# alexbuburuzan/MObI

Measured on AMD Instinct MI355X. Metric: denoising throughput (UNet element-forwards/s = steps/s x UNet batch), higher is better.
Workload: dtype bf16; 1 GPU; mobi_nusc_512 UNet denoising step, 8 objects/GPU (UNet batch 16), latent 64x64, DDIM-50 schedule, cfg_scale 1.0; objects_per_gpu=8, unet_batch=16, latent=64, sampler=ddim, parallelism=dp1 (objects sharded, no collective in the loop)

## Files before the change

mobi_amd/csrc/igemm.hip:

```cpp
#include <stdlib.h>

#include <type_traits>

#include "common.h"
#include "tuning.h"
#include "igemm_small.h"

#ifndef MOBI_FRAG2
#define MOBI_FRAG2 0
#endif
#ifndef MOBI_DMA_KS
#define MOBI_DMA_KS 1
#endif
#if defined(MOBI_IGEMM_FENCE) && MOBI_IGEMM_FENCE
#define MOBI_SCHED_FENCE() __builtin_amdgcn_sched_barrier(0)
#else
#define MOBI_SCHED_FENCE() ((void)0)
#endif

#ifndef MOBI_DBG_SKIP
#define MOBI_DBG_SKIP 0
#endif
#ifndef MOBI_PP_DMA_KS
#define MOBI_PP_DMA_KS 1
// ... 515 lines not shown

template <typename T, int NT, bool GEGLU, bool VEC = true>
__device__ __forceinline__ int direct_epilogue(const IgemmArgs& a, f32x4 (&acc)[NT][4], DirectEpiRegs<NT>& q, int lane,
                                               int group, int nw0, int mw0) {
  const int r16 = lane & 15, g4 = lane >> 4;
  const float scale = a.scale;
  T* __restrict__ outT = reinterpret_cast<T*>(a.out);
  const bool has_vec = VEC && (a.bias || a.rowvec);
  if (has_vec) {
#pragma unroll
    for (int ni = 0; ni < NT; ++ni) asm volatile("" : "+v"(q.bias[ni]));
  }
  if (!GEGLU && a.residual) {
#pragma unroll
    for (int ni = 0; ni < NT; ++ni) { asm volatile("" : "+v"(q.res[ni][0])); asm volatile("" : "+v"(q.res[ni][1])); }
  }
  constexpr bool geglu = GEGLU;
#pragma unroll
  for (int p = 0; p < 2; ++p) {
    const int mi = geglu ? 2 * p + (g4 >> 1) : 2 * p + (g4 & 1);
    const int m = mw0 + mi * 16 + r16;
    const int img = m / a.hw_out, rem = m - img * a.hw_out;
    T* rowp = outT + (long long)(group * a.imgs_per_group + img) * a.out_img_stride + (long long)rem * a.cout;
#pragma unroll
    for (int ni = 0; ni < NT; ++ni) {
      f32x4 x = acc[ni][2 * p] * scale, y = acc[ni][2 * p + 1] * scale;
      if (has_vec) {
        const f32x4 b = __builtin_bit_cast(f32x4, q.bias[ni]);
        x += b; y += b;
      }
      float xs[4] = {x[0], x[1], x[2], x[3]}, ys[4] = {y[0], y[1], y[2], y[3]};
      if constexpr (geglu) MOBI_SWAP4("v_permlane32_swap_b32", xs, ys);
      else MOBI_SWAP4("v_permlane16_swap_b32", xs, ys);
      if constexpr (geglu) {
        float o[4];
#pragma unroll
        for (int r = 0; r < 4; ++r) o[r] = xs[r] * gelu_erf_f(ys[r]);
        vm_store8(rowp + (nw0 >> 1) + ni * 8 + 4 * (g4 & 1), pack4<T>(o));
      } else {
        float o[8] = {xs[0], xs[1], xs[2], xs[3], ys[0], ys[1], ys[2], ys[3]};
        if (a.residual) {
          float rf[8];
          unpack8<T>(q.res[ni][p], rf);
#pragma unroll
          for (int j = 0; j < 8; ++j) o[j] += rf[j];
        }
        vm_store16(rowp + nw0 + ni * 16 + 8 * (g4 >> 1), pack8<T>(o));
      }
    }
  }
  return 2 * NT;
}

template <typename T, int NT, bool GEGLU>
__device__ __forceinline__ void ring_register_epilogue(const IgemmArgs& a, f32x4 (&acc)[NT][8], int lane, int group, int nw0,
                                                       int mw0) {
  const int r16 = lane & 15, g4 = lane >> 4;
  T* __restrict__ outT = reinterpret_cast<T*>(a.out);
  const T* __restrict__ resid = reinterpret_cast<const T*>(a.residual);
  const bool has_res = !GEGLU && a.residual;
  u32x4 res[2][NT];
#pragma unroll
  for (int ni = 0; ni < NT; ++ni) res[0][ni] = res[1][ni] = u32x4{0u, 0u, 0u, 0u};
  auto out_row = [&](int k) {
    const int mi = GEGLU ? 2 * k + (g4 >> 1) : 2 * k + (g4 & 1);
    return mw0 + mi * 16 + r16;
  };
  auto request_res = [&](int k, u32x4 (&r)[NT]) {
    const int m = out_row(k);
    const int img = m / a.hw_out, rem = m - img * a.hw_out;
    const T* rowp = resid + (long long)(group * a.imgs_per_group + img) * a.res_img_stride + (long long)rem * a.cout + nw0 +
                    8 * (g4 >> 1);
#pragma unroll
    for (int ni = 0; ni < NT; ++ni) r[ni] = vm_load16(rowp + ni * 16);
  };
  if (has_res) request_res(0, res[0]);
#pragma unroll
  for (int k = 0; k < 4; ++k) {
    if (has_res) {
      if (k + 1 < 4) request_res(k + 1, res[(k + 1) & 1]);
      const bool both = k > 0 && k + 1 < 4;
      if (both) { if (NT == 5) asm volatile("s_waitcnt vmcnt(10)" ::: "memory"); else asm volatile("s_waitcnt vmcnt(8)" ::: "memory"); }
      else                  { if (NT == 5) asm volatile("s_waitcnt vmcnt(5)" ::: "memory"); else asm volatile("s_waitcnt vmcnt(4)" ::: "memory"); }
    }
    if constexpr (!GEGLU) {
#pragma unroll
      for (int ni = 0; ni < NT; ++ni) asm volatile("" : "+v"(res[k & 1][ni]));
    }
    const int m = out_row(k);
    const int img = m / a.hw_out, rem = m - img * a.hw_out;
    T* rowp = outT + (long long)(group * a.imgs_per_group + img) * a.out_img_stride + (long long)rem * a.cout;
#pragma unroll
    for (int ni = 0; ni < NT; ++ni) {
      const f32x4 x = acc[ni][2 * k], y = acc[ni][2 * k + 1];
      float xs[4] = {x[0], x[1], x[2], x[3]}, ys[4] = {y[0], y[1], y[2], y[3]};
      if constexpr (GEGLU) MOBI_SWAP4("v_permlane32_swap_b32", xs, ys);
      else MOBI_SWAP4("v_permlane16_swap_b32", xs, ys);
      if constexpr (GEGLU) {
        float o[4];
#pragma unroll
        for (int r = 0; r < 4; ++r) o[r] = xs[r] * gelu_erf_f(ys[r]);
        vm_store8(rowp + (nw0 >> 1) + ni * 8 + 4 * (g4 & 1), pack4<T>(o));
      } else {
        float o[8] = {xs[0], xs[1], xs[2], xs[3], ys[0], ys[1], ys[2], ys[3]};
        if (has_res) {
          float rf[8];
          unpack8<T>(res[k & 1][ni], rf);
#pragma unroll
          for (int j = 0; j < 8; ++j) o[j] += rf[j];
        }
        vm_store16(rowp + nw0 + ni * 16 + 8 * (g4 >> 1), pack8<T>(o));
      }
    }
  }
}

template <int NT>
struct PpEpiRegs {
  u32x4 res0[NT];
};
template <typename T, int NT>
__device__ __forceinline__ void pp_residual_request(const IgemmArgs& a, u32x4 (&r)[NT], int p, int lane, int group,
                                                    int nw0, int mw0) {
  const int r16 = lane & 15, g4 = lane >> 4;
  const T* __restrict__ resid = reinterpret_cast<const T*>(a.residual);
  const int m = mw0 + (2 * p + (g4 & 1)) * 16 + r16;
  const int img = m >> a.hw_shift, rem = m & (a.hw_out - 1);
  const T* rowp = resid + (long long)(group * a.imgs_per_group + img) * a.res_img_stride + (long long)rem * a.cout +
                  nw0 + 8 * (g4 >> 1);
#pragma unroll
  for (int ni = 0; ni < NT; ++ni) r[ni] = vm_load16(rowp + ni * 16);
}
#ifndef MOBI_PP_RES0_EARLY
#define MOBI_PP_RES0_EARLY 0
#endif
template <typename T, int NT, bool GEGLU>
__device__ __forceinline__ int pp_epilogue_request(const IgemmArgs& a, PpEpiRegs<NT>& q, int lane, int group, int nw0,
                                                   int mw0) {
  if (!MOBI_PP_RES0_EARLY || GEGLU || !a.residual) return 0;
  pp_residual_request<T, NT>(a, q.res0, 0, lane, group, nw0, mw0);
  return NT;
}
template <typename T, int NT, bool GEGLU>
__device__ __forceinline__ int pp_epilogue(const IgemmArgs& a, f32x4 (&acc)[NT][4], PpEpiRegs<NT>& q, int lane, int group,
                                           int nw0, int mw0) {
  const int r16 = lane & 15, g4 = lane >> 4;
  T* __restrict__ outT = reinterpret_cast<T*>(a.out);
  const bool resid = !GEGLU && a.residual;
  u32x4 res1[NT];
  int n_issued = 0;
  if (resid) {
    if (!MOBI_PP_RES0_EARLY) {
      pp_residual_request<T, NT>(a, q.res0, 0, lane, group, nw0, mw0);
      n_issued += NT;
    }
    pp_residual_request<T, NT>(a, res1, 1, lane, group, nw0, mw0);
    n_issued += NT;
    if (!MOBI_PP_RES0_EARLY) {
      if (NT == 5) asm volatile("s_waitcnt vmcnt(5)" ::: "memory"); else asm volatile("s_waitcnt vmcnt(4)" ::: "memory");
    }
#pragma unroll
    for (int ni = 0; ni < NT; ++ni) asm volatile("" : "+v"(q.res0[ni]));
  }
#pragma unroll
// ... 954 lines not shown
  MOBI_STAMP_AT(2);
  wait_vmcnt_le(vm_issued - mk_req);
  finish_tile(p_nw0, p_mw0);
  if constexpr (SLAB) {
    if (a.sync) {
      const int L = xcd_remap(blockIdx.x, nblk);
      MOBI_TILE_OF_M(L, ftm, ftn);
      splitk_arrive_and_finish<T, 512>(a, L, ftm * BM, BM, ftn * BN, BN, &s_arrive);
    }
  }
#if MOBI_STAMP
  asm volatile("s_waitcnt vmcnt(0)" ::: "memory");
  MOBI_STAMP_AT(3);
  if (g_stamps && threadIdx.x == 0) {
    unsigned long long* d = g_stamps + (size_t)(blockIdx.x + gridDim.x * (blockIdx.y + gridDim.y * blockIdx.z)) * 8;
    d[5] = (unsigned long long)nk;
    d[6] = (unsigned long long)((nblk - (int)blockIdx.x + (int)gridDim.x - 1) / (int)gridDim.x);
  }
#endif
#if MOBI_STAMP == 3
  if (g_phase && lane == 0) {
    unsigned long long* d = g_phase + ((size_t)(blockIdx.x + gridDim.x * (blockIdx.y + gridDim.y * blockIdx.z)) * 8 + wave) * 16;
    for (int i = 0; i < 8; ++i) d[i] = pp_acc[i >> 2][i & 3];
    d[8] = pp_n;
  }
#endif
#undef MOBI_PP_T
#undef MOBI_PP_BARRIER
}

typedef _Float16 f16x2_t __attribute__((ext_vector_type(2)));
typedef __bf16 bf16x2_t __attribute__((ext_vector_type(2)));
__device__ __forceinline__ void rowstat_acc(const f16x8& x, float& sum, float& sq) {
  struct Q { f16x2_t p[4]; };
  const Q q = __builtin_bit_cast(Q, x);
  const f16x2_t one = {(_Float16)1.0f, (_Float16)1.0f};
#pragma unroll
  for (int i = 0; i < 4; ++i) {
    sum = __builtin_amdgcn_fdot2(q.p[i], one, sum, false);
    sq = __builtin_amdgcn_fdot2(q.p[i], q.p[i], sq, false);
  }
}
__device__ __forceinline__ void rowstat_acc(const bf16x8& x, float& sum, float& sq) {
  struct Q { bf16x2_t p[4]; };
  const Q q = __builtin_bit_cast(Q, x);
  const bf16x2_t one = {(__bf16)1.0f, (__bf16)1.0f};
#pragma unroll
  for (int i = 0; i < 4; ++i) {
    sum = __builtin_amdgcn_fdot2_f32_bf16(q.p[i], one, sum, false);
    sq = __builtin_amdgcn_fdot2_f32_bf16(q.p[i], q.p[i], sq, false);
  }
}

template <int NT, int MT, int SPW>
__device__ __forceinline__ void ln_fold_acc(const IgemmArgs& a, f32x4 (&acc)[NT][MT], const float (&ls_sum)[SPW],
                                            const float (&ls_sq)[SPW], float* s_rowstat, int lane, int wm, int wn, int nw0,
                                            bool add_bias) {
  const int r16 = lane & 15, g4 = lane >> 4;
  const float inv_k = 1.0f / (float)a.ktot;
#pragma unroll
  for (int i = 0; i < SPW; ++i) {
    float sm = ls_sum[i], sq = ls_sq[i];
    sm += __shfl_xor(sm, 16, 64); sq += __shfl_xor(sq, 16, 64);
    sm += __shfl_xor(sm, 32, 64); sq += __shfl_xor(sq, 32, 64);
    const float mean = sm * inv_k;
    const float var = fmaxf(sq * inv_k - mean * mean, 0.f);
    if (g4 == 0) {
      float* d = s_rowstat + ((wm * MT + SPW * wn + i) * 16 + r16) * 2;
      d[0] = mean; d[1] = rsqrtf(var + a.ln_eps);
    }
  }
  __syncthreads();
#pragma unroll
  for (int ni = 0; ni < NT; ++ni) {
    const int n = nw0 + ni * 16 + g4 * 4;
    f32x4 sv = f32x4{0.f, 0.f, 0.f, 0.f}, bv = f32x4{0.f, 0.f, 0.f, 0.f};
    if (n < a.n_packed) {
      sv = *reinterpret_cast<const f32x4*>(a.ln_svec + n);
      if (add_bias && a.bias) bv = *reinterpret_cast<const f32x4*>(a.bias + n);
    }
#pragma unroll
    for (int mi = 0; mi < MT; ++mi) {
      const float* d = s_rowstat + ((wm * MT + mi) * 16 + r16) * 2;
      const float mean = d[0], rstd = d[1];
      acc[ni][mi] = rstd * (acc[ni][mi] - mean * sv) + bv;
    }
  }
}

template <typename T, int NT, bool TR, int NW, int MT, bool LNF = false, bool LEAKY = false>
__global__ __launch_bounds__(NW * 64, 2) void igemm_ring_kernel(const IgemmArgs a) {
  typedef typename Vec8<T>::type frag_t;
  constexpr bool WIDE = NW == 8;
  constexpr int BM = 2 * MT * 16;
  constexpr int APW = BM / 16 / NW;
  constexpr int WAVE_N = NT * 16;
  constexpr int BN = (NW / 2) * WAVE_N;
  constexpr int WPIECES = BN / 16;
  constexpr int SLOT = (BM + BN) * 64;
  constexpr int RING = 4 * SLOT;
  constexpr int STAGE_BYTES = EpiGeom<32, TR, NT>::BYTES;
  constexpr int LDS_BYTES = RING > NW * STAGE_BYTES ? RING : NW * STAGE_BYTES;
  constexpr unsigned OOB = 0x80000000u;
  __shared__ __attribute__((aligned(16))) unsigned char lds[LDS_BYTES];
  __shared__ int s_arrive;
  __shared__ float s_rowstat[LNF ? BM * 2 : 2];
  static_assert(!(LNF && TR), "the LayerNorm fold has no transposed-output form");
  typedef __attribute__((address_space(3))) void* lds_ptr_t;

  const int tid = threadIdx.x, lane = tid & 63, wave = tid >> 6;
  const int wave_s = __builtin_amdgcn_readfirstlane(wave);
  const int wm = wave & 1, wn = wave >> 1;
  const int group = blockIdx.z;
  const int nblk = a.tiles_m * a.tiles_n;
  const int L = xcd_remap(blockIdx.x, nblk);
  MOBI_TILE_OF(L, tile_m, tile_n);
  const int m0 = tile_m * BM, n0 = tile_n * BN;
  constexpr int SPW = MT / (NW / 2);
  constexpr bool lnf = LNF;
  float ls_sum[SPW], ls_sq[SPW];
#pragma unroll
  for (int i = 0; i < SPW; ++i) ls_sum[i] = ls_sq[i] = 0.f;
  MOBI_STAMP_AT(0);
  const bool w_tiled = a.w_tiled != nullptr;
  const T* wgt = (w_tiled ? reinterpret_cast<const T*>(a.w_tiled) : reinterpret_cast<const T*>(a.weight)) + (long long)group * a.w_group_stride;
  const __amdgpu_buffer_rsrc_t rx0 = __builtin_amdgcn_make_buffer_rsrc(const_cast<void*>(a.src0), 0, a.src0_bytes, 0x00020000);
  const __amdgpu_buffer_rsrc_t rx1 =
      __builtin_amdgcn_make_buffer_rsrc(const_cast<void*>(a.src1 ? a.src1 : a.src0), 0, a.src1 ? a.src1_bytes : 0, 0x00020000);
  const __amdgpu_buffer_rsrc_t rw = __builtin_amdgcn_make_buffer_rsrc(const_cast<T*>(wgt), 0, a.w_bytes, 0x00020000);

  const int rp = lane >> 2;
  const unsigned perm = (0x1320u >> (((rp >> 2) & 3) * 4)) & 3u;
  const unsigned chunk16 = (((unsigned)lane & 3u) ^ perm) * 16u;
  int x_base[APW], x_h[APW], x_w[APW];
  bool x_ok[APW];
#pragma unroll
  for (int j = 0; j < APW; ++j) {
    const int m = m0 + 16 * (APW * wave + j) + rp;
    x_ok[j] = m < a.M;
    const int mm = x_ok[j] ? m : 0;
    const int img = mm / a.hw_out, rem = mm - img * a.hw_out;
    const int ho = rem / a.wout, wo = rem - ho * a.wout;
    x_base[j] = (group * a.imgs_per_group + img) * a.img_pix_stride;
    x_h[j] = ho * a.stride - a.pad_h;
    x_w[j] = wo * a.stride - a.pad_w;
  }
  unsigned w_off[3];
#pragma unroll
  for (int i = 0; i < 3; ++i) {
    const int piece = wave + NW * i;
    const int n = n0 + 16 * piece + rp;
    w_off[i] = (piece < WPIECES && n < a.n_packed) ? (unsigned)n * (unsigned)a.ktot * 2u + chunk16 : OOB;
    if (w_tiled) w_off[i] = (piece < WPIECES && n0 + 16 * piece < a.n_packed)
                                ? (unsigned)(n0 / 16 + piece) * (unsigned)(a.ktot >> 5) * 1024u + (unsigned)lane * 16u : OOB;
  }
  const int hlog = a.hin << a.up, wlog = a.win << a.up;
  const int ks_all = a.ktot >> 5;
  const int ks_begin = blockIdx.y * a.nk_per * 2;
  const int ks_end = min(ks_all, ks_begin + a.nk_per * 2);
  int u_c, u_tap, u_ky, u_kx;
  {
    const long long c_first = (long long)ks_begin * 32;
    u_tap = (int)(c_first / a.C); u_c = (int)(c_first - (long long)u_tap * a.C);
    u_ky = u_tap / a.kw; u_kx = u_tap - u_ky * a.kw;
  }
  unsigned f_row[APW];
#pragma unroll
  for (int j = 0; j < APW; ++j) f_row[j] = OOB;
  int f_tap = -1, f_src = -1, f_ks = ks_begin;

  auto issue_step = [&]() {
    unsigned char* st = lds + (f_ks & 3) * SLOT;
    const bool live = f_ks < ks_end;
    const int src = u_c >= a.c0 ? 1 : 0;
    if (live && (u_tap != f_tap || src != f_src)) {
      f_tap = u_tap; f_src = src;
      const unsigned cs2 = (unsigned)(src ? a.c1 : a.c0) * 2u;
#pragma unroll
      for (int j = 0; j < APW; ++j) {
        const int hi = x_h[j] + u_ky, wi = x_w[j] + u_kx;
        const bool ok = x_ok[j] && (unsigned)hi < (unsigned)hlog && (unsigned)wi < (unsigned)wlog;
        f_row[j] = ok ? (unsigned)(x_base[j] + (hi >> a.up) * a.win + (wi >> a.up)) * cs2 + chunk16 : OOB;
      }
    }
    const int soff = (src ? u_c - a.c0 : u_c) * 2;
#pragma unroll
    for (int j = 0; j < APW; ++j) {
      const unsigned vo = live ? f_row[j] : OOB;
      if (src) __builtin_amdgcn_raw_ptr_buffer_load_lds(rx1, (lds_ptr_t)(st + 16 * (APW * wave_s + j) * 64), 16, vo, soff, 0, 0);
      else     __builtin_amdgcn_raw_ptr_buffer_load_lds(rx0, (lds_ptr_t)(st + 16 * (APW * wave_s + j) * 64), 16, vo, soff, 0, 0);
    }
    const int kb = w_tiled ? f_ks * 1024 : f_ks * 64;
#pragma unroll
    for (int i = 0; i < 3; ++i) {
      if (i == 2 && (NT != 5 || wave_s >= NW / 2)) break;
      const unsigned vo = live ? w_off[i] : OOB;
      __builtin_amdgcn_raw_ptr_buffer_load_lds(rw, (lds_ptr_t)(st + BM * 64 + (wave_s + NW * i) * 1024), 16, vo, kb, 0, 0);
    }
    ++f_ks;
    if (live) {
      u_c += 32;
      if (u_c >= a.C) { u_c = 0; ++u_tap; if (++u_kx == a.kw) { u_kx = 0; ++u_ky; } }
    }
  };
  auto wait_step = [&]() {
    if (NT == 5 && wave_s < NW / 2) {
      if (APW == 2) asm volatile("s_waitcnt vmcnt(10)" ::: "memory"); else asm volatile("s_waitcnt vmcnt(8)" ::: "memory");
    } else {
      if (APW == 2) asm volatile("s_waitcnt vmcnt(8)" ::: "memory"); else asm volatile("s_waitcnt vmcnt(6)" ::: "memory");
    }
  };

  f32x4 acc[NT][MT];
#pragma unroll
  for (int i = 0; i < NT; ++i)
#pragma unroll
    for (int j = 0; j < MT; ++j) acc[i][j] = f32x4{0.f, 0.f, 0.f, 0.f};

  const int r16 = lane & 15, g4 = lane >> 4;
  if constexpr (WIDE && MT == 8 && !TR) {
    if (!lnf && a.ring_direct && (a.bias || a.rowvec)) {
      const float* vec = a.bias;
      if (a.rowvec) {
        const int img = __builtin_amdgcn_readfirstlane((m0 + wm * 128) / a.hw_out);
        vec = a.rowvec + (long long)(group * a.imgs_per_group + img) * a.rowvec_stride;
      }
#pragma unroll
      for (int i = 0; i < NT; ++i) {
        const f32x4 b = *reinterpret_cast<const f32x4*>(vec + n0 + wn * WAVE_N + i * 16 + g4 * 4);
#pragma unroll
        for (int j = 0; j < MT; ++j) acc[i][j] = b;
      }
    }
  }
  const unsigned fsw = (((unsigned)g4 ^ ((0x1320u >> (((r16 >> 2) & 3) * 4)) & 3u)) << 4);
  const unsigned char* xrd = lds + (wm * MT * 16 + r16) * 64 + fsw;
  const unsigned char* wrd = lds + BM * 64 + (wn * WAVE_N + r16) * 64 + fsw;

  auto read_frags = [&](int s, frag_t (&xf)[MT], frag_t (&wf)[NT]) {
    const int so = (s & 3) * SLOT;
#pragma unroll
    for (int mi = 0; mi < MT; ++mi) xf[mi] = __builtin_bit_cast(frag_t, ld16(xrd + so + mi * 16 * 64));
#pragma unroll
    for (int ni = 0; ni < NT; ++ni) wf[ni] = __builtin_bit_cast(frag_t, ld16(wrd + so + ni * 16 * 64));
  };
  auto multiply = [&](const frag_t (&xf)[MT], const frag_t (&wf)[NT]) {
    __builtin_amdgcn_s_setprio(1);
#pragma unroll
    for (int ni = 0; ni < NT; ++ni)
#pragma unroll
      for (int mi = 0; mi < MT; ++mi)
        acc[ni][mi] = TR ? mfma16(xf[mi], wf[ni], acc[ni][mi]) : mfma16(wf[ni], xf[mi], acc[ni][mi]);
    __builtin_amdgcn_s_setprio(0);
  };
  auto multiply_stats = [&](const frag_t (&xf)[MT], const frag_t (&wf)[NT], auto wnc) {
    constexpr int WNC = decltype(wnc)::value;
    __builtin_amdgcn_s_setprio(1);
#pragma unroll
    for (int ni = 0; ni < NT; ++ni)
#pragma unroll
      for (int mi = 0; mi < MT; ++mi) {
        acc[ni][mi] = TR ? mfma16(xf[mi], wf[ni], acc[ni][mi]) : mfma16(wf[ni], xf[mi], acc[ni][mi]);
        if (ni == 0 && mi < SPW) rowstat_acc(xf[SPW * WNC + mi], ls_sum[mi], ls_sq[mi]);
      }
#pragma unroll
    for (int i = 0; i < 8 * SPW; ++i) {
      __builtin_amdgcn_sched_group_barrier(0x008, 2, 0);
      __builtin_amdgcn_sched_group_barrier(0x002, 1, 0);
    }
#pragma unroll
    for (int i = 0; i < SPW; ++i) asm volatile("" : "+v"(ls_sum[i]), "+v"(ls_sq[i]));
    __builtin_amdgcn_s_setprio(0);
  };
#define MOBI_RING_BARRIER()                   \
  do {                                        \
    __builtin_amdgcn_sched_barrier(0);        \
    __builtin_amdgcn_s_barrier();             \
    __builtin_amdgcn_sched_barrier(0);        \
  } while (0)

  issue_step(); issue_step(); issue_step();
  auto k_loop = [&](auto wnc) {
  if constexpr (WIDE && MOBI_RING_STAGGER) {
    const bool late = wave_s >= NW / 2;
    wait_step();
    MOBI_STAMP_AT(1);
    if (late) MOBI_RING_BARRIER();
#if MOBI_STAMP == 4
    unsigned long long wp_t[8], wp_acc[7] = {0, 0, 0, 0, 0, 0, 0};
#define MOBI_WP(i) wp_t[i] = __builtin_amdgcn_s_memtime()
#else
#define MOBI_WP(i) ((void)0)
#endif
#pragma clang loop unroll(disable)
    for (int s = ks_begin; s < ks_end; ++s) {
      MOBI_WP(0);
      MOBI_RING_BARRIER();
      MOBI_WP(1);
      frag_t xf[MT], wf[NT];
      read_frags(s, xf, wf);
      __builtin_amdgcn_sched_barrier(0);
      issue_step();
      __builtin_amdgcn_sched_barrier(0);
      MOBI_WP(2);
      asm volatile("s_waitcnt lgkmcnt(0)" ::: "memory");
      MOBI_WP(3);
      if (late) wait_step();
      MOBI_WP(4);
      MOBI_RING_BARRIER();
      MOBI_WP(5);
      if constexpr (lnf) multiply_stats(xf, wf, wnc); else multiply(xf, wf);
#if MOBI_STAMP == 4
      asm volatile("s_nop 0" ::: "memory");
#endif
      MOBI_WP(6);
      if (!late) wait_step();
#if MOBI_STAMP == 4
      MOBI_WP(7);
      if (s > ks_begin) for (int i = 0; i < 7; ++i) wp_acc[i] += wp_t[i + 1] - wp_t[i];
#endif
    }
#if MOBI_STAMP == 4
    if (g_phase && lane == 0) {
      unsigned long long* d = g_phase + ((size_t)(blockIdx.x + gridDim.x * (blockIdx.y + gridDim.y * blockIdx.z)) * 8 + wave) * 8;
      for (int i = 0; i < 7; ++i) d[i] = wp_acc[i];
      d[7] = (unsigned long long)(ks_end - ks_begin - 1);
    }
#endif
#undef MOBI_WP
    if (!late) MOBI_RING_BARRIER();
  } else {
#if MOBI_STAMP == 4
    unsigned long long rp_t[6], rp_acc[5] = {0, 0, 0, 0, 0};
#define MOBI_RP(i) rp_t[i] = __builtin_amdgcn_s_memtime()
#else
#define MOBI_RP(i) ((void)0)
#endif
#pragma clang loop unroll(disable)
    for (int s = ks_begin; s < ks_end; ++s) {
      MOBI_RP(0);
      wait_step();
      MOBI_RP(1);
      MOBI_RING_BARRIER();
      MOBI_RP(2);
      frag_t xf[MT], wf[NT];
      read_frags(s, xf, wf);
      __builtin_amdgcn_sched_barrier(0);
      issue_step();
      __builtin_amdgcn_sched_barrier(0);
      MOBI_RP(3);
      asm volatile("s_waitcnt lgkmcnt(0)" ::: "memory");
      MOBI_RP(4);
      if constexpr (lnf) multiply_stats(xf, wf, wnc); else multiply(xf, wf);
#if MOBI_STAMP == 4
      asm volatile("s_nop 0" ::: "memory");
      MOBI_RP(5);
      if (s > ks_begin) for (int i = 0; i < 5; ++i) rp_acc[i] += rp_t[i + 1] - rp_t[i];
#endif
    }
#if MOBI_STAMP == 4
    if (g_phase && lane == 0) {
      unsigned long long* d = g_phase + ((size_t)(blockIdx.x + gridDim.x * (blockIdx.y + gridDim.y * blockIdx.z)) * 8 + wave) * 8;
      for (int i = 0; i < 5; ++i) d[i] = rp_acc[i];
      d[5] = (unsigned long long)(ks_end - ks_begin - 1);
    }
#endif
#undef MOBI_RP
  }
  };
  if constexpr (lnf) {
    const int wn_s = wave_s >> 1;
    if (wn_s == 0) k_loop(std::integral_constant<int, 0>{});
    else if (wn_s == 1 || NW == 4) k_loop(std::integral_constant<int, 1>{});
    else if (wn_s == 2) k_loop(std::integral_constant<int, NW == 8 ? 2 : 0>{});
    else k_loop(std::integral_constant<int, NW == 8 ? 3 : 0>{});
  } else {
    k_loop(std::integral_constant<int, 0>{});
  }
#undef MOBI_RING_BARRIER
  MOBI_STAMP_AT(2);
  if constexpr (lnf) {
    ln_fold_acc<NT, MT, SPW>(a, acc, ls_sum, ls_sq, s_rowstat, lane, wm, wave_s >> 1, n0 + wn * WAVE_N,
                             WIDE && MT == 8 && a.ring_direct);
  }
  if constexpr (MT == 4 && !TR && !LEAKY) {
    if (a.sm_direct) {
      asm volatile("s_waitcnt vmcnt(0)" ::: "memory");
      const int nw0 = n0 + wn * WAVE_N, mw0 = m0 + wm * 64;
      if (a.split_ws) {
        float* wsp = a.split_ws + (long long)blockIdx.y * a.M * a.n_packed;
#pragma unroll
        for (int mi = 0; mi < 4; ++mi) {
          float* rowp = wsp + (long long)(mw0 + mi * 16 + r16) * a.n_packed + nw0 + g4 * 4;
#pragma unroll
          for (int ni = 0; ni < NT; ++ni) slab_store16(a.sync_mode == 1, rowp + ni * 16, __builtin_bit_cast(u32x4, acc[ni][mi]));
        }
        if (a.sync) {
          splitk_arrive_and_finish<T, NW * 64>(a, tile_m * a.tiles_n + tile_n, m0, BM, n0, BN, &s_arrive);
        }
      } else {
        DirectEpiRegs<NT> q;
#pragma unroll
        for (int ni = 0; ni < NT; ++ni) { q.bias[ni] = u32x4{0u, 0u, 0u, 0u}; q.res[ni][0] = q.res[ni][1] = u32x4{0u, 0u, 0u, 0u}; }
        direct_epilogue_request<T, NT>(a, q, lane, group, nw0, mw0);
        asm volatile("s_waitcnt vmcnt(0)" ::: "memory");
        if (a.epilogue == MOBI_EPI_GEGLU) direct_epilogue<T, NT, true>(a, acc, q, lane, group, nw0, mw0);
        else direct_epilogue<T, NT, false>(a, acc, q, lane, group, nw0, mw0);
      }
      return;
    }
  }
  if constexpr (WIDE && MT == 8 && !TR && !LEAKY) {
    if (a.ring_direct) {
      asm volatile("s_waitcnt vmcnt(0)" ::: "memory");
      if constexpr (MT == 8) {
        if (a.epilogue == MOBI_EPI_GEGLU) ring_register_epilogue<T, NT, true>(a, acc, lane, group, n0 + wn * WAVE_N, m0 + wm * 128);
        else ring_register_epilogue<T, NT, false>(a, acc, lane, group, n0 + wn * WAVE_N, m0 + wm * 128);
      }
#if MOBI_STAMP
      asm volatile("s_waitcnt vmcnt(0)" ::: "memory");
      MOBI_STAMP_AT(3);
      if (g_stamps && threadIdx.x == 0) {
        unsigned long long* d = g_stamps + (size_t)(blockIdx.x + gridDim.x * (blockIdx.y + gridDim.y * blockIdx.z)) * 8;
        unsigned hw, xcc;
        asm volatile("s_getreg_b32 %0, hwreg(HW_REG_HW_ID)" : "=s"(hw));
        asm volatile("s_getreg_b32 %0, hwreg(HW_REG_XCC_ID)" : "=s"(xcc));
        d[4] = ((unsigned long long)xcc << 32) | hw;
        d[5] = (unsigned long long)(ks_end - ks_begin);
        d[6] = 1;
      }
#endif
      return;
    }
  }
  asm volatile("s_waitcnt vmcnt(0)" ::: "memory");
  __syncthreads();
  float* stage = reinterpret_cast<float*>(lds) + wave * (STAGE_BYTES / 4);
#pragma unroll
  for (int h = 0; h < MT / 4; ++h) {
    f32x4 part[NT][4];
#pragma unroll
    for (int i = 0; i < NT; ++i)
#pragma unroll
      for (int j = 0; j < 4; ++j) part[i][j] = acc[i][4 * h + j];
    igemm_epilogue<T, NT, TR, 32, MT == 4, LEAKY>(a, stage, part, lane, group, n0 + wn * WAVE_N, m0 + wm * MT * 16 + 64 * h);
  }
  if constexpr (!TR) {
    if (a.split_ws && a.sync) {
      splitk_arrive_and_finish<T, NW * 64>(a, tile_m * a.tiles_n + tile_n, m0, BM, n0, BN, &s_arrive);
    }
  }
#if MOBI_STAMP
  asm volatile("s_waitcnt vmcnt(0)" ::: "memory");
  MOBI_STAMP_AT(3);
  if (g_stamps && threadIdx.x == 0) {
    unsigned long long* d = g_stamps + (size_t)(blockIdx.x + gridDim.x * (blockIdx.y + gridDim.y * blockIdx.z)) * 8;
    unsigned hw, xcc;
    asm volatile("s_getreg_b32 %0, hwreg(HW_REG_HW_ID)" : "=s"(hw));
    asm volatile("s_getreg_b32 %0, hwreg(HW_REG_XCC_ID)" : "=s"(xcc));
    d[4] = ((unsigned long long)xcc << 32) | hw;
    d[5] = (unsigned long long)(ks_end - ks_begin);
    d[6] = 1;
  }
#endif
}

template <typename T, int NT, bool TR, bool LNF = false, bool OVL = false>
__global__ __launch_bounds__(256, 1) void igemm_ring64_kernel(const IgemmArgs a) {
  typedef typename Vec8<T>::type frag_t;
  constexpr int NW = 4, MT = 4, BM = 128, SL = 4;
  constexpr int APW = BM / 8 / NW;
  constexpr int WAVE_N = NT * 16;
  constexpr int BN = 2 * WAVE_N;
  constexpr int SLOT = (BM + BN) * 128;
  constexpr int RING = SL * SLOT;
  constexpr int STAGE_BYTES = EpiGeom<32, TR, NT>::BYTES;
  constexpr int LDS_BYTES = RING > NW * STAGE_BYTES ? RING : NW * STAGE_BYTES;
  constexpr unsigned OOB = 0x80000000u;
  constexpr int TAIL_BYTES = OVL ? 16 + (LNF ? BM * 2 * 4 : 0) : 0;
  __shared__ __attribute__((aligned(16))) unsigned char lds[LDS_BYTES + TAIL_BYTES];
  __shared__ int s_arrive_obj;
  __shared__ float s_rowstat_obj[LNF ? BM * 2 : 2];
  int* const s_arrive = OVL ? reinterpret_cast<int*>(lds + LDS_BYTES) : &s_arrive_obj;
  float* const s_rowstat = OVL ? reinterpret_cast<float*>(lds + LDS_BYTES + 16) : s_rowstat_obj;
  static_assert(!(LNF && TR), "the LayerNorm fold has no transposed-output form");
  typedef __attribute__((address_space(3))) void* lds_ptr_t;

  MOBI_SP_ENTRY;
  const int tid = threadIdx.x, lane = tid & 63, wave = tid >> 6;
  const int wave_s = __builtin_amdgcn_readfirstlane(wave);
  const int wm = wave & 1, wn = wave >> 1;
  const int group = blockIdx.z;
  const int nblk = a.tiles_m * a.tiles_n;
  const int L = xcd_remap(blockIdx.x, nblk);
  MOBI_TILE_OF(L, tile_m, tile_n);
  const int m0 = tile_m * BM, n0 = tile_n * BN;
  const T* wgt = reinterpret_cast<const T*>(a.weight) + (long long)group * a.w_group_stride;
  const __amdgpu_buffer_rsrc_t rx0 = __builtin_amdgcn_make_buffer_rsrc(const_cast<void*>(a.src0), 0, a.src0_bytes, 0x00020000);
  const __amdgpu_buffer_rsrc_t rx1 =
      __builtin_amdgcn_make_buffer_rsrc(const_cast<void*>(a.src1 ? a.src1 : a.src0), 0, a.src1 ? a.src1_bytes : 0, 0x00020000);
  const __amdgpu_buffer_rsrc_t rw = __builtin_amdgcn_make_buffer_rsrc(const_cast<T*>(wgt), 0, a.w_bytes, 0x00020000);

  const int rp = lane >> 3;
  const unsigned chunk16 = (unsigned)((lane & 7) ^ rp) * 16u;
  int x_base[APW], x_h[APW], x_w[APW];
  bool x_ok[APW];
#pragma unroll
  for (int j = 0; j < APW; ++j) {
    const int m = m0 + 8 * (APW * wave + j) + rp;
    x_ok[j] = m < a.M;
    const int mm = x_ok[j] ? m : 0;
    const int img = mm / a.hw_out, rem = mm - img * a.hw_out;
    const int ho = rem / a.wout, wo = rem - ho * a.wout;
    x_base[j] = (group * a.imgs_per_group + img) * a.img_pix_stride;
    x_h[j] = ho * a.stride - a.pad_h;
    x_w[j] = wo * a.stride - a.pad_w;
  }
// ... 299 lines not shown
      st16(outT + off, pack8<T>(o));
    }
  }
}

static int compute_units() {
  if (tuning().persist_blocks > 0) return tuning().persist_blocks;
  static int cached[64] = {0};
  int dev = 0;
  if (hipGetDevice(&dev) != hipSuccess || dev < 0 || dev >= 64) return 256;
  if (!cached[dev]) {
    int n = 0;
    if (hipDeviceGetAttribute(&n, hipDeviceAttributeMultiprocessorCount, dev) != hipSuccess || n <= 0) n = 256;
    cached[dev] = n;
  }
  return cached[dev];
}

template <typename T>
static int launch_splitk_reduce(const IgemmArgs& a, hipStream_t st) {
  long long blocks = ((long long)a.M * (a.cout >> 3) + 255) / 256;
  if (blocks > 4096) blocks = 4096;
  hipLaunchKernelGGL((igemm_splitk_reduce_kernel<T>), dim3((unsigned)blocks), dim3(256), 0, st, a);
  MOBI_CHECK_LAUNCH();
  return MOBI_OK;
}

template <typename T>
static int launch_igemm(const mobi_igemm_params* p, const IgemmArgs& a, int groups, hipStream_t st) {
  const bool tr = p->out_mode == MOBI_OUT_TRANSPOSED;
  const bool nt5 = (a.n_packed % 160) == 0;
  dim3 grid(a.tiles_m * a.tiles_n, a.splits, groups);
#define MOBI_IGEMM_LAUNCH(NT_, TR_, WM_, FAST_) \
  hipLaunchKernelGGL((igemm_kernel<T, NT_, TR_, WM_, FAST_>), grid, dim3(128 * WM_), 0, st, a)
#ifdef MOBI_DEV
#define MOBI_IGEMM_BY_FAST(NT_, TR_, WM_) \
  do { if (a.fast) MOBI_IGEMM_LAUNCH(NT_, TR_, WM_, true); else MOBI_IGEMM_LAUNCH(NT_, TR_, WM_, false); } while (0)
#else
#define MOBI_IGEMM_BY_FAST(NT_, TR_, WM_) MOBI_IGEMM_LAUNCH(NT_, TR_, WM_, false)
#endif
#define MOBI_IGEMM_BY_TR(NT_, WM_) \
  do { if (tr) MOBI_IGEMM_BY_FAST(NT_, true, WM_); else MOBI_IGEMM_BY_FAST(NT_, false, WM_); } while (0)
  if (a.epilogue == MOBI_EPI_LEAKY_RELU) {
    if (a.wide == 2) {
      if (nt5) hipLaunchKernelGGL((igemm_ring_kernel<T, 5, false, 8, 8, false, true>), grid, dim3(512), 0, st, a);
      else     hipLaunchKernelGGL((igemm_ring_kernel<T, 4, false, 8, 8, false, true>), grid, dim3(512), 0, st, a);
    } else {
      if (nt5) hipLaunchKernelGGL((igemm_ring_kernel<T, 5, false, 4, 4, false, true>), grid, dim3(256), 0, st, a);
      else     hipLaunchKernelGGL((igemm_ring_kernel<T, 4, false, 4, 4, false, true>), grid, dim3(256), 0, st, a);
    }
  }
  else if (a.wide == 2) {
#define MOBI_W2_LAUNCH(NT_, TR_) hipLaunchKernelGGL((igemm_ring_kernel<T, NT_, TR_, 8, 8>), grid, dim3(512), 0, st, a)
    if (a.ln_svec) {
      if (nt5) hipLaunchKernelGGL((igemm_ring_kernel<T, 5, false, 8, 8, true>), grid, dim3(512), 0, st, a);
      else     hipLaunchKernelGGL((igemm_ring_kernel<T, 4, false, 8, 8, true>), grid, dim3(512), 0, st, a);
    }
    else if (nt5) { if (tr) MOBI_W2_LAUNCH(5, true); else MOBI_W2_LAUNCH(5, false); }
    else     { if (tr) MOBI_W2_LAUNCH(4, true); else MOBI_W2_LAUNCH(4, false); }
#undef MOBI_W2_LAUNCH
  }
  else if (a.wide == 1) {
    if (nt5) hipLaunchKernelGGL((igemm_ring_kernel<T, 5, false, 8, 4>), grid, dim3(512), 0, st, a);
    else     hipLaunchKernelGGL((igemm_ring_kernel<T, 4, false, 8, 4>), grid, dim3(512), 0, st, a);
  }
  else if (a.wm == 4 && a.fast && a.glds && a.pp) {
    dim3 block(512);
    dim3 pgrid(grid.x < (unsigned)compute_units() ? grid.x : (unsigned)compute_units(), grid.y, grid.z);
    if (a.split_ws) {
      if (nt5) hipLaunchKernelGGL((igemm_pp_kernel<T, 5, false, true>), pgrid, block, 0, st, a);
      else     hipLaunchKernelGGL((igemm_pp_kernel<T, 4, false, true>), pgrid, block, 0, st, a);
    } else {
#define MOBI_PP_LAUNCH(NT_, G_) hipLaunchKernelGGL((igemm_pp_kernel<T, NT_, G_>), pgrid, block, 0, st, a)
      if (a.epilogue == MOBI_EPI_GEGLU) { if (nt5) MOBI_PP_LAUNCH(5, true); else MOBI_PP_LAUNCH(4, true); }
      else                              { if (nt5) MOBI_PP_LAUNCH(5, false); else MOBI_PP_LAUNCH(4, false); }
#undef MOBI_PP_LAUNCH
    }
  }
#ifdef MOBI_DEV
  else if (a.wm == 4 && a.fast && a.glds) {
    dim3 block(512);
    dim3 pgrid(grid.x < (unsigned)compute_units() ? grid.x : (unsigned)compute_units(), grid.y, grid.z);
    const int mode = tr ? 1 : (a.epi_direct ? (a.epilogue == MOBI_EPI_GEGLU ? 3 : 2) : 0);
#define MOBI_GLDS_LAUNCH(NT_, MODE_) hipLaunchKernelGGL((igemm_glds_kernel<T, NT_, MODE_>), pgrid, block, 0, st, a)
#define MOBI_GLDS_BY_MODE(NT_)                                                                     \
  do { switch (mode) { case 0: MOBI_GLDS_LAUNCH(NT_, 0); break; case 1: MOBI_GLDS_LAUNCH(NT_, 1); break; \
                       case 2: MOBI_GLDS_LAUNCH(NT_, 2); break; default: MOBI_GLDS_LAUNCH(NT_, 3); break; } } while (0)
    if (nt5) MOBI_GLDS_BY_MODE(5); else MOBI_GLDS_BY_MODE(4);
#undef MOBI_GLDS_BY_MODE
#undef MOBI_GLDS_LAUNCH
  }
#endif
  else if (a.wm == 4) { if (nt5) MOBI_IGEMM_BY_TR(5, 4); else MOBI_IGEMM_BY_TR(4, 4); }
  else if (a.sm && a.sm64) {
#define MOBI_SM64_LAUNCH_W(NT_, TR_, LNF_, OVL_) \
  hipLaunchKernelGGL((igemm_ring64_kernel<T, NT_, TR_, LNF_, OVL_>), grid, dim3(256), 0, st, a)
#define MOBI_SM64_LAUNCH(NT_, TR_, LNF_) \
  do { if (tuning().sm64_ovl != 0) MOBI_SM64_LAUNCH_W(NT_, TR_, LNF_, true); else MOBI_SM64_LAUNCH_W(NT_, TR_, LNF_, false); } while (0)
    if (a.ln_svec) { if (nt5) MOBI_SM64_LAUNCH(5, false, true); else MOBI_SM64_LAUNCH(4, false, true); }
    else if (nt5) { if (tr) MOBI_SM64_LAUNCH(5, true, false); else MOBI_SM64_LAUNCH(5, false, false); }
    else     { if (tr) MOBI_SM64_LAUNCH(4, true, false); else MOBI_SM64_LAUNCH(4, false, false); }
#undef MOBI_SM64_LAUNCH
#undef MOBI_SM64_LAUNCH_W
  }
  else if (a.sm) {
#define MOBI_SM_LAUNCH(NT_, TR_) hipLaunchKernelGGL((igemm_ring_kernel<T, NT_, TR_, 4, 4>), grid, dim3(256), 0, st, a)
    if (a.ln_svec) {
// ... 351 lines not shown
```

mobi_amd/csrc/tuning.h:

```cpp
#pragma once
namespace mobi {
struct Tuning {
  int persist_blocks;
  int pp_split;
  int wm;
  int fast;
  int glds;
  int lin;
  int epi_direct;
  int pp;
  int sm;
  int wide;
  int wide128;
  int ring_direct;
  int sm_direct;
  int w_tiled;
  int n_major;
  int sm64;
  int sm64_ovl;
  int split_target;
  int fused_split;
  int split_longk;
  int split_round4;
  int attn_bwd_exact_d;
  int small;
  int small_mflop;
  int small_conv_m;
  int tka_mfma;
  int attn_nw;
  int attn_sp;
  int tka_rows;
  int attn_nw8_blocks;
  int attn_h16;
  int attn_xcd;
  int cout_mfma;
  int skinny_mfma;
  int gn_coop;
  int gn_fused;
  int gn_split_pw4;
  int attn_v3;
};
const Tuning& tuning();
}
```

mobi_amd/csrc/tuning.hip:

```cpp
#include <atomic>
#include <cstdlib>
#include <mutex>

#include "common.h"
#include "tuning.h"

namespace mobi {
namespace {
Tuning g_tuning;
std::once_flag g_once;

int env_int(const char* name) {
  const char* e = getenv(name);
  return (e && e[0]) ? atoi(e) : -1;
}
void read_env() {
  g_tuning.persist_blocks = env_int("MOBI_IGEMM_PERSIST_BLOCKS");
  g_tuning.pp_split = env_int("MOBI_IGEMM_PP_SPLIT");
  g_tuning.wm = env_int("MOBI_IGEMM_WM");
  g_tuning.fast = env_int("MOBI_IGEMM_FAST");
  g_tuning.glds = env_int("MOBI_IGEMM_GLDS");
  g_tuning.lin = env_int("MOBI_IGEMM_LIN");
  g_tuning.epi_direct = env_int("MOBI_IGEMM_EPI_DIRECT");
  g_tuning.pp = env_int("MOBI_IGEMM_PP");
  g_tuning.sm = env_int("MOBI_IGEMM_SM");
  g_tuning.wide = env_int("MOBI_IGEMM_WIDE");
  g_tuning.wide128 = env_int("MOBI_IGEMM_WIDE128");
  g_tuning.ring_direct = env_int("MOBI_IGEMM_RING_DIRECT");
  g_tuning.sm_direct = env_int("MOBI_IGEMM_SM_DIRECT");
  g_tuning.w_tiled = env_int("MOBI_IGEMM_WTILED");
  g_tuning.sm64 = env_int("MOBI_IGEMM_SM64");
  g_tuning.sm64_ovl = env_int("MOBI_IGEMM_SM64_OVL");
  g_tuning.n_major = env_int("MOBI_IGEMM_N_MAJOR");
  g_tuning.split_target = env_int("MOBI_IGEMM_SPLIT_TARGET");
  g_tuning.split_longk = env_int("MOBI_IGEMM_SPLIT_LONGK");
  g_tuning.split_round4 = env_int("MOBI_IGEMM_SPLIT_ROUND4");
  g_tuning.attn_bwd_exact_d = env_int("MOBI_ATTN_BWD_EXACT_D");
  g_tuning.fused_split = env_int("MOBI_IGEMM_FUSED_SPLIT");
  g_tuning.small = env_int("MOBI_IGEMM_SMALL");
  g_tuning.small_mflop = env_int("MOBI_IGEMM_SMALL_MFLOP");
  g_tuning.small_conv_m = env_int("MOBI_IGEMM_SMALL_CONV_M");
  g_tuning.tka_mfma = env_int("MOBI_TKA_MFMA");
  g_tuning.attn_nw = env_int("MOBI_ATTN_NW");
  g_tuning.attn_sp = env_int("MOBI_ATTN_SP");
  g_tuning.attn_v3 = env_int("MOBI_ATTN_V3");
  g_tuning.gn_fused = env_int("MOBI_GN_FUSED");
  g_tuning.gn_coop = env_int("MOBI_GN_COOP");
  g_tuning.gn_split_pw4 = env_int("MOBI_GN_SPLIT_PW4");
  g_tuning.skinny_mfma = env_int("MOBI_SKINNY_MFMA");
  g_tuning.cout_mfma = env_int("MOBI_COUT_MFMA");
  g_tuning.attn_xcd = env_int("MOBI_ATTN_XCD");
  g_tuning.attn_h16 = env_int("MOBI_ATTN_H16");
  g_tuning.attn_nw8_blocks = env_int("MOBI_ATTN_NW8_BLOCKS");
  g_tuning.tka_rows = env_int("MOBI_TKA_ROWS");
}
}

const Tuning& tuning() {
  std::call_once(g_once, read_env);
  return g_tuning;
}
}

extern "C" int mobi_tuning_reload(void) {
  std::call_once(mobi::g_once, [] {});
  mobi::read_env();
  return MOBI_OK;
}

extern "C" int mobi_build_info(void) {
#ifdef MOBI_DEV
  return 1;
#else
  return 0;
#endif
}
```

Measured before the change: 817.4 UNet element-forwards/s.

## Add persistent tile-walking ring igemm kernel that prefetches the next tile across seams

Adds a PERSIST variant of the wide ring implicit-GEMM kernel. It is launched with one block per compute unit, and each block walks several output tiles in sequence. While the current tile's K-loop runs, the LDS ring is pre-filled with the next tile's first K-steps, using per-seam vmcnt waits and a rolling slot offset. This is meant to hide the fill and epilogue bubbles between tiles. It is enabled by default for non-residual, ungrouped, unsplit 1x1 layers whose grid exceeds the CU count. The cost is more complex hand-tuned wait counts and a fixed persistent grid that may balance load worse than the hardware scheduler.

```diff
diff --git a/mobi_amd/csrc/igemm.hip b/mobi_amd/csrc/igemm.hip
--- a/mobi_amd/csrc/igemm.hip
+++ b/mobi_amd/csrc/igemm.hip
@@ -591,13 +591,13 @@
   return 2 * NT;
 }
 
-template <typename T, int NT, bool GEGLU>
+template <typename T, int NT, bool GEGLU, bool RES = true>
 __device__ __forceinline__ void ring_register_epilogue(const IgemmArgs& a, f32x4 (&acc)[NT][8], int lane, int group, int nw0,
                                                        int mw0) {
   const int r16 = lane & 15, g4 = lane >> 4;
   T* __restrict__ outT = reinterpret_cast<T*>(a.out);
   const T* __restrict__ resid = reinterpret_cast<const T*>(a.residual);
-  const bool has_res = !GEGLU && a.residual;
+  const bool has_res = RES && !GEGLU && a.residual;
   u32x4 res[2][NT];
 #pragma unroll
   for (int ni = 0; ni < NT; ++ni) res[0][ni] = res[1][ni] = u32x4{0u, 0u, 0u, 0u};
@@ -622,7 +622,7 @@
       if (both) { if (NT == 5) asm volatile("s_waitcnt vmcnt(10)" ::: "memory"); else asm volatile("s_waitcnt vmcnt(8)" ::: "memory"); }
       else                  { if (NT == 5) asm volatile("s_waitcnt vmcnt(5)" ::: "memory"); else asm volatile("s_waitcnt vmcnt(4)" ::: "memory"); }
     }
-    if constexpr (!GEGLU) {
+    if constexpr (!GEGLU && RES) {
 #pragma unroll
       for (int ni = 0; ni < NT; ++ni) asm volatile("" : "+v"(res[k & 1][ni]));
     }
@@ -639,7 +639,8 @@
         float o[4];
 #pragma unroll
         for (int r = 0; r < 4; ++r) o[r] = xs[r] * gelu_erf_f(ys[r]);
-        vm_store8(rowp + (nw0 >> 1) + ni * 8 + 4 * (g4 & 1), pack4<T>(o));
+        if constexpr (RES) vm_store8(rowp + (nw0 >> 1) + ni * 8 + 4 * (g4 & 1), pack4<T>(o));
+        else vm_store8(rowp + ((nw0 >> 1) + ni * 8 + 4 * (g4 & 1)), pack4<T>(o));
       } else {
         float o[8] = {xs[0], xs[1], xs[2], xs[3], ys[0], ys[1], ys[2], ys[3]};
         if (has_res) {
@@ -648,7 +649,8 @@
 #pragma unroll
           for (int j = 0; j < 8; ++j) o[j] += rf[j];
         }
-        vm_store16(rowp + nw0 + ni * 16 + 8 * (g4 >> 1), pack8<T>(o));
+        if constexpr (RES) vm_store16(rowp + nw0 + ni * 16 + 8 * (g4 >> 1), pack8<T>(o));
+        else vm_store16(rowp + (nw0 + ni * 16 + 8 * (g4 >> 1)), pack8<T>(o));
       }
     }
   }
@@ -1709,12 +1711,14 @@
   }
 }
 
-template <int NT, int MT, int SPW>
+template <int NT, int MT, int SPW, bool RAW_BARRIER = false>
 __device__ __forceinline__ void ln_fold_acc(const IgemmArgs& a, f32x4 (&acc)[NT][MT], const float (&ls_sum)[SPW],
                                             const float (&ls_sq)[SPW], float* s_rowstat, int lane, int wm, int wn, int nw0,
                                             bool add_bias) {
   const int r16 = lane & 15, g4 = lane >> 4;
-  const float inv_k = 1.0f / (float)a.ktot;
+  int k_i = a.ktot;
+  if constexpr (RAW_BARRIER) asm volatile("" : "+s"(k_i));
+  const float inv_k = 1.0f / (float)k_i;
 #pragma unroll
   for (int i = 0; i < SPW; ++i) {
     float sm = ls_sum[i], sq = ls_sq[i];
@@ -1727,7 +1731,13 @@
       d[0] = mean; d[1] = rsqrtf(var + a.ln_eps);
     }
   }
-  __syncthreads();
+  if constexpr (RAW_BARRIER) {
+    asm volatile("s_waitcnt lgkmcnt(0)" ::: "memory");
+    __builtin_amdgcn_s_barrier();
+    asm volatile("" ::: "memory");
+  } else {
+    __syncthreads();
+  }
 #pragma unroll
   for (int ni = 0; ni < NT; ++ni) {
     const int n = nw0 + ni * 16 + g4 * 4;
@@ -1745,10 +1755,11 @@
   }
 }
 
-template <typename T, int NT, bool TR, int NW, int MT, bool LNF = false, bool LEAKY = false>
+template <typename T, int NT, bool TR, int NW, int MT, bool LNF = false, bool LEAKY = false, bool PERSIST = false>
 __global__ __launch_bounds__(NW * 64, 2) void igemm_ring_kernel(const IgemmArgs a) {
   typedef typename Vec8<T>::type frag_t;
   constexpr bool WIDE = NW == 8;
+  static_assert(!PERSIST || (NW == 8 && MT == 8 && !TR && !LEAKY), "the tile walk exists for the register epilogue of the 256-pixel tiles");
   constexpr int BM = 2 * MT * 16;
   constexpr int APW = BM / 16 / NW;
   constexpr int WAVE_N = NT * 16;
@@ -1767,12 +1778,15 @@
 
   const int tid = threadIdx.x, lane = tid & 63, wave = tid >> 6;
   const int wave_s = __builtin_amdgcn_readfirstlane(wave);
-  const int wm = wave & 1, wn = wave >> 1;
+  const int wm = PERSIST ? (wave_s & 1) : (wave & 1), wn = PERSIST ? (wave_s >> 1) : (wave >> 1);
   const int group = blockIdx.z;
   const int nblk = a.tiles_m * a.tiles_n;
-  const int L = xcd_remap(blockIdx.x, nblk);
-  MOBI_TILE_OF(L, tile_m, tile_n);
-  const int m0 = tile_m * BM, n0 = tile_n * BN;
+  int tile_m, tile_n, m0, n0;
+  {
+    const int L = xcd_remap(blockIdx.x, nblk);
+    MOBI_TILE_OF(L, tm_, tn_);
+    tile_m = tm_; tile_n = tn_; m0 = tm_ * BM; n0 = tn_ * BN;
+  }
   constexpr int SPW = MT / (NW / 2);
   constexpr bool lnf = LNF;
   float ls_sum[SPW], ls_sq[SPW];
@@ -1791,10 +1805,16 @@
   const unsigned chunk16 = (((unsigned)lane & 3u) ^ perm) * 16u;
   int x_base[APW], x_h[APW], x_w[APW];
   bool x_ok[APW];
+  unsigned w_off[3];
+  auto fetch_rows = [&](int fm0, int fn0) {
+  const int wv = PERSIST ? wave_s : wave;
+  int ln = lane;
+  if constexpr (PERSIST) asm volatile("" : "+v"(ln));
+  const int rp = ln >> 2;
 #pragma unroll
   for (int j = 0; j < APW; ++j) {
-    const int m = m0 + 16 * (APW * wave + j) + rp;
-    x_ok[j] = m < a.M;
+    const int m = fm0 + 16 * (APW * wv + j) + rp;
+    x_ok[j] = PERSIST || m < a.M;
     const int mm = x_ok[j] ? m : 0;
     const int img = mm / a.hw_out, rem = mm - img * a.hw_out;
     const int ho = rem / a.wout, wo = rem - ho * a.wout;
@@ -1802,15 +1822,16 @@
     x_h[j] = ho * a.stride - a.pad_h;
     x_w[j] = wo * a.stride - a.pad_w;
   }
-  unsigned w_off[3];
 #pragma unroll
   for (int i = 0; i < 3; ++i) {
-    const int piece = wave + NW * i;
-    const int n = n0 + 16 * piece + rp;
+    const int piece = wv + NW * i;
+    const int n = fn0 + 16 * piece + rp;
     w_off[i] = (piece < WPIECES && n < a.n_packed) ? (unsigned)n * (unsigned)a.ktot * 2u + chunk16 : OOB;
-    if (w_tiled) w_off[i] = (piece < WPIECES && n0 + 16 * piece < a.n_packed)
-                                ? (unsigned)(n0 / 16 + piece) * (unsigned)(a.ktot >> 5) * 1024u + (unsigned)lane * 16u : OOB;
-  }
+    if (w_tiled) w_off[i] = (piece < WPIECES && fn0 + 16 * piece < a.n_packed)
+                                ? (unsigned)(fn0 / 16 + piece) * (unsigned)(a.ktot >> 5) * 1024u + (unsigned)ln * 16u : OOB;
+  }
+  };
+  fetch_rows(m0, n0);
   const int hlog = a.hin << a.up, wlog = a.win << a.up;
   const int ks_all = a.ktot >> 5;
   const int ks_begin = blockIdx.y * a.nk_per * 2;
@@ -1825,9 +1846,23 @@
 #pragma unroll
   for (int j = 0; j < APW; ++j) f_row[j] = OOB;
   int f_tap = -1, f_src = -1, f_ks = ks_begin;
+  int f_slot = ks_begin;
+  int f_bid = blockIdx.x;
+  auto fetch_next_tile = [&]() {
+    if (f_ks < ks_end || f_bid >= nblk) return;
+    f_bid += (int)gridDim.x;
+    if (f_bid >= nblk) return;
+    const int Lf = xcd_remap(f_bid, nblk);
+    MOBI_TILE_OF(Lf, ftm, ftn);
+    fetch_rows(ftm * BM, ftn * BN);
+    const long long c_first = (long long)ks_begin * 32;
+    u_tap = (int)(c_first / a.C); u_c = (int)(c_first - (long long)u_tap * a.C);
+    u_ky = u_tap / a.kw; u_kx = u_tap - u_ky * a.kw;
+    f_tap = -1; f_src = -1; f_ks = ks_begin;
+  };
 
   auto issue_step = [&]() {
-    unsigned char* st = lds + (f_ks & 3) * SLOT;
+    unsigned char* st = lds + ((PERSIST ? f_slot : f_ks) & 3) * SLOT;
     const bool live = f_ks < ks_end;
     const int src = u_c >= a.c0 ? 1 : 0;
     if (live && (u_tap != f_tap || src != f_src)) {
@@ -1855,6 +1890,7 @@
       __builtin_amdgcn_raw_ptr_buffer_load_lds(rw, (lds_ptr_t)(st + BM * 64 + (wave_s + NW * i) * 1024), 16, vo, kb, 0, 0);
     }
     ++f_ks;
+    if constexpr (PERSIST) ++f_slot;
     if (live) {
       u_c += 32;
       if (u_c >= a.C) { u_c = 0; ++u_tap; if (++u_kx == a.kw) { u_kx = 0; ++u_ky; } }
@@ -1867,14 +1903,39 @@
       if (APW == 2) asm volatile("s_waitcnt vmcnt(8)" ::: "memory"); else asm volatile("s_waitcnt vmcnt(6)" ::: "memory");
     }
   };
+  auto wait_step_seam = [&]() {
+    static_assert(!PERSIST || APW == 2, "counts of the 256-pixel tiles");
+    if (NT == 5 && wave_s < NW / 2) asm volatile("s_waitcnt vmcnt(30)" ::: "memory");
+    else if (NT == 5) asm volatile("s_waitcnt vmcnt(28)" ::: "memory");
+    else asm volatile("s_waitcnt vmcnt(24)" ::: "memory");
+  };
+  int seam = 0;
+  int late_s = wave_s >> 2;
+  if constexpr (PERSIST) asm volatile("" : "+s"(late_s));
+  int g_off = 0;
 
   f32x4 acc[NT][MT];
+  if constexpr (PERSIST) {
+    issue_step(); fetch_next_tile(); issue_step(); fetch_next_tile(); issue_step();
+  }
+  for (int bid = blockIdx.x;;) {
+  int lane_t = lane;
+  if constexpr (PERSIST) {
+    asm volatile("" : "+v"(lane_t));
+    if (seam) {
+      const int L = xcd_remap(bid, nblk);
+      MOBI_TILE_OF(L, tm_, tn_);
+      tile_m = tm_; tile_n = tn_; m0 = tm_ * BM; n0 = tn_ * BN;
+#pragma unroll
+      for (int i = 0; i < SPW; ++i) ls_sum[i] = ls_sq[i] = 0.f;
+    }
+  }
 #pragma unroll
   for (int i = 0; i < NT; ++i)
 #pragma unroll
     for (int j = 0; j < MT; ++j) acc[i][j] = f32x4{0.f, 0.f, 0.f, 0.f};
 
-  const int r16 = lane & 15, g4 = lane >> 4;
+  const int r16 = lane_t & 15, g4 = lane_t >> 4;
   if constexpr (WIDE && MT == 8 && !TR) {
     if (!lnf && a.ring_direct && (a.bias || a.rowvec)) {
       const float* vec = a.bias;
@@ -1890,12 +1951,12 @@
       }
     }
   }
-  const unsigned fsw = (((unsigned)g4 ^ ((0x1320u >> (((r16 >> 2) & 3) * 4)) & 3u)) << 4);
-  const unsigned char* xrd = lds + (wm * MT * 16 + r16) * 64 + fsw;
-  const unsigned char* wrd = lds + BM * 64 + (wn * WAVE_N + r16) * 64 + fsw;
+  const unsigned fsw = (((unsigned)(lane >> 4) ^ ((0x1320u >> ((((lane & 15) >> 2) & 3) * 4)) & 3u)) << 4);
+  const unsigned char* xrd = lds + (wm * MT * 16 + (lane & 15)) * 64 + fsw;
+  const unsigned char* wrd = lds + BM * 64 + (wn * WAVE_N + (lane & 15)) * 64 + fsw;
 
   auto read_frags = [&](int s, frag_t (&xf)[MT], frag_t (&wf)[NT]) {
-    const int so = (s & 3) * SLOT;
+    const int so = ((PERSIST ? s + g_off : s) & 3) * SLOT;
 #pragma unroll
     for (int mi = 0; mi < MT; ++mi) xf[mi] = __builtin_bit_cast(frag_t, ld16(xrd + so + mi * 16 * 64));
 #pragma unroll
@@ -1936,9 +1997,31 @@
     __builtin_amdgcn_sched_barrier(0);        \
   } while (0)
 
-  issue_step(); issue_step(); issue_step();
+  if constexpr (!PERSIST) { issue_step(); issue_step(); issue_step(); }
   auto k_loop = [&](auto wnc) {
-  if constexpr (WIDE && MOBI_RING_STAGGER) {
+  if constexpr (PERSIST) {
+    static_assert(!PERSIST || MOBI_RING_STAGGER, "the tile walk is written for the staggered loop");
+    auto is_late = [&]() { int l = late_s; asm volatile("" : "+s"(l)); return l != 0; };
+    if (seam) wait_step_seam(); else wait_step();
+    if (is_late()) MOBI_RING_BARRIER();
+#pragma clang loop unroll(disable)
+    for (int s = ks_begin; s < ks_end; ++s) {
+      const int young = seam & (int)(s < ks_begin + 2);
+      MOBI_RING_BARRIER();
+      fetch_next_tile();
+      frag_t xf[MT], wf[NT];
+      read_frags(s, xf, wf);
+      __builtin_amdgcn_sched_barrier(0);
+      issue_step();
+      __builtin_amdgcn_sched_barrier(0);
+      asm volatile("s_waitcnt lgkmcnt(0)" ::: "memory");
+      if (is_late()) { if (young) wait_step_seam(); else wait_step(); }
+      MOBI_RING_BARRIER();
+      if constexpr (lnf) multiply_stats(xf, wf, wnc); else multiply(xf, wf);
+      if (!is_late()) { if (young) wait_step_seam(); else wait_step(); }
+    }
+    if (!is_late()) MOBI_RING_BARRIER();
+  } else if constexpr (WIDE && MOBI_RING_STAGGER) {
     const bool late = wave_s >= NW / 2;
     wait_step();
     MOBI_STAMP_AT(1);
@@ -2036,9 +2119,20 @@
   }
 #undef MOBI_RING_BARRIER
   MOBI_STAMP_AT(2);
+  int lane_e = lane;
+  if constexpr (PERSIST) asm volatile("" : "+v"(lane_e));
   if constexpr (lnf) {
-    ln_fold_acc<NT, MT, SPW>(a, acc, ls_sum, ls_sq, s_rowstat, lane, wm, wave_s >> 1, n0 + wn * WAVE_N,
-                             WIDE && MT == 8 && a.ring_direct);
+    ln_fold_acc<NT, MT, SPW, PERSIST>(a, acc, ls_sum, ls_sq, s_rowstat, lane_e, wm, wave_s >> 1, n0 + wn * WAVE_N,
+                                      WIDE && MT == 8 && a.ring_direct);
+  }
+  if constexpr (PERSIST) {
+    if (a.epilogue == MOBI_EPI_GEGLU) ring_register_epilogue<T, NT, true, false>(a, acc, lane_e, group, n0 + wn * WAVE_N, m0 + wm * 128);
+    else ring_register_epilogue<T, NT, false, false>(a, acc, lane_e, group, n0 + wn * WAVE_N, m0 + wm * 128);
+    bid += (int)gridDim.x;
+    if (bid >= nblk) break;
+    g_off += ks_end - ks_begin;
+    seam = 1;
+    continue;
   }
   if constexpr (MT == 4 && !TR && !LEAKY) {
     if (a.sm_direct) {
@@ -2120,6 +2214,23 @@
     d[6] = 1;
   }
 #endif
+  break;
+  }
+  if constexpr (PERSIST) {
+    asm volatile("s_waitcnt vmcnt(0)" ::: "memory");
+#if MOBI_STAMP
+    MOBI_STAMP_AT(3);
+    if (g_stamps && threadIdx.x == 0) {
+      unsigned long long* d = g_stamps + (size_t)(blockIdx.x + gridDim.x * (blockIdx.y + gridDim.y * blockIdx.z)) * 8;
+      unsigned hw, xcc;
+      asm volatile("s_getreg_b32 %0, hwreg(HW_REG_HW_ID)" : "=s"(hw));
+      asm volatile("s_getreg_b32 %0, hwreg(HW_REG_XCC_ID)" : "=s"(xcc));
+      d[4] = ((unsigned long long)xcc << 32) | hw;
+      d[5] = (unsigned long long)(ks_end - ks_begin);
+      d[6] = (unsigned long long)((nblk - (int)blockIdx.x + (int)gridDim.x - 1) / (int)gridDim.x);
+    }
+#endif
+  }
 }
 
 template <typename T, int NT, bool TR, bool LNF = false, bool OVL = false>
@@ -2525,7 +2636,16 @@
   }
   else if (a.wide == 2) {
 #define MOBI_W2_LAUNCH(NT_, TR_) hipLaunchKernelGGL((igemm_ring_kernel<T, NT_, TR_, 8, 8>), grid, dim3(512), 0, st, a)
-    if (a.ln_svec) {
+    const int cus = compute_units();
+    if (a.ring_direct && !tr && !a.residual && !a.split_ws && groups == 1 && a.splits == 1 && grid.x > (unsigned)cus &&
+        tuning().ring_persist != 0 && (a.kh * a.kw == 1 || tuning().ring_persist == 2)) {
+      const dim3 wgrid((unsigned)cus, 1, 1);
+#define MOBI_W2_WALK(NT_, LNF_) hipLaunchKernelGGL((igemm_ring_kernel<T, NT_, false, 8, 8, LNF_, false, true>), wgrid, dim3(512), 0, st, a)
+      if (a.ln_svec) { if (nt5) MOBI_W2_WALK(5, true); else MOBI_W2_WALK(4, true); }
+      else           { if (nt5) MOBI_W2_WALK(5, false); else MOBI_W2_WALK(4, false); }
+#undef MOBI_W2_WALK
+    }
+    else if (a.ln_svec) {
       if (nt5) hipLaunchKernelGGL((igemm_ring_kernel<T, 5, false, 8, 8, true>), grid, dim3(512), 0, st, a);
       else     hipLaunchKernelGGL((igemm_ring_kernel<T, 4, false, 8, 8, true>), grid, dim3(512), 0, st, a);
     }
diff --git a/mobi_amd/csrc/tuning.h b/mobi_amd/csrc/tuning.h
--- a/mobi_amd/csrc/tuning.h
+++ b/mobi_amd/csrc/tuning.h
@@ -18,6 +18,7 @@
   int n_major;
   int sm64;
   int sm64_ovl;
+  int ring_persist;
   int split_target;
   int fused_split;
   int split_longk;
diff --git a/mobi_amd/csrc/tuning.hip b/mobi_amd/csrc/tuning.hip
--- a/mobi_amd/csrc/tuning.hip
+++ b/mobi_amd/csrc/tuning.hip
@@ -31,6 +31,7 @@
   g_tuning.w_tiled = env_int("MOBI_IGEMM_WTILED");
   g_tuning.sm64 = env_int("MOBI_IGEMM_SM64");
   g_tuning.sm64_ovl = env_int("MOBI_IGEMM_SM64_OVL");
+  g_tuning.ring_persist = env_int("MOBI_IGEMM_RING_PERSIST");
   g_tuning.n_major = env_int("MOBI_IGEMM_N_MAJOR");
   g_tuning.split_target = env_int("MOBI_IGEMM_SPLIT_TARGET");
   g_tuning.split_longk = env_int("MOBI_IGEMM_SPLIT_LONGK");
```

Measured after the change: 816.9 UNet element-forwards/s. No clear change (-0.1%).
